# dalab/matrix-manifolds

Hardware: AMD Instinct MI355X
Metric: pairwise manifold-dist/sec (fwd+bwd), SPD(3) 5k-node (higher is better)
Workload: dtype f32; 1 GPU; grqc-class graph, n=5000 nodes -> SPD(3) affine-invariant, all 12497500 pairs, squared distance + backward, reference init (||log X||=0.1); parallelism=pair-rows sharded x1, 1 all-reduce, launch=hipGraph replay (kernels)

## Files before the change

matrix-manifolds_amd/csrc/spd_pair.hpp:

```cpp
#pragma once
#include <hip/hip_runtime.h>

#include "../../include/mm_manifolds.h"
#include "prof.hpp"
#include <algorithm>
#include <climits>
#include <cstdint>
#include <cstdlib>
#include <type_traits>

#include "smallmat.hpp"
#include "loss.hpp"
#include "adam.hpp"
#include "spd_rules.hpp"

#include "spd_ws.hpp"
#include "spd_step.hpp"
#include "stamp.hpp"

namespace mm {

template <typename T, int D>
__device__ __forceinline__ void node_tables(const T (&xs)[Packed<D>::NP], int i, T* __restrict__ nodeL, T* __restrict__ nodeX,
                                            T* __restrict__ nodeC, int* __restrict__ bad, T* __restrict__ nodeLd,
// ... 125 lines not shown
  }
  T s = T(0);
#pragma unroll
  for (int k = 0; k < D; ++k) {
    w[k] = Num<T>::min(Num<T>::max(ev[k], wmin), wmax);
    lw[k] = Num<T>::log(w[k]);
    s = Num<T>::fma(lw[k], lw[k], s);
    if (rho) rho[k] = w[k] == ev[k] ? T(1) : ev[k] * Num<T>::rcp(w[k]);
  }
  return s;
}

template <typename T, int D> __device__ __forceinline__ T frob2(const T (&m)[Packed<D>::NP]) {
  T s = T(0);
#pragma unroll
  for (int r = 0; r < D; ++r) {
    s = Num<T>::fma(m[pidx(r, r)], m[pidx(r, r)], s);
#pragma unroll
    for (int c = 0; c < r; ++c) s = Num<T>::fma(T(2) * m[pidx(r, c)], m[pidx(r, c)], s);
  }
  return s;
}
template <typename T, int D> __device__ __forceinline__ T close_gate(const T (&a)[Packed<D>::NP]) {
  using N = Num<T>;
  T e[Packed<D>::NP];
#pragma unroll
  for (int k = 0; k < Packed<D>::NP; ++k) e[k] = a[k];
#pragma unroll
  for (int r = 0; r < D; ++r) e[pidx(r, r)] -= T(1);
  if constexpr (D == 3) {
    return N::fma(e[0], e[0], N::fma(e[1], e[1], e[3] * e[3])) + N::fma(e[1], e[1], N::fma(e[2], e[2], e[4] * e[4])) +
           N::fma(e[3], e[3], N::fma(e[4], e[4], e[5] * e[5]));
  } else {
    T p2 = T(0);
#pragma unroll
    for (int r = 0; r < D; ++r) {
      T acc = e[pidx(r, 0)] * e[pidx(0, r)];
#pragma unroll
      for (int k = 1; k < D; ++k) acc = N::fma(e[pidx(r, k)], e[pidx(k, r)], acc);
      p2 += acc;
    }
    return p2;
  }
}
constexpr double kCloseGate = 0.09;
template <typename T, int D> __device__ __forceinline__ void log_close(const T (&a)[Packed<D>::NP], T (&m0)[Packed<D>::NP],
                                                                     T pre = T(1)) {
  if constexpr (D == 3) log_series3<T>(a, m0, pre); else log_series4<T>(a, m0, pre);
}
template <typename T, int D> __device__ __forceinline__ T log_cayley(const T (&a)[Packed<D>::NP], T (&m0)[Packed<D>::NP], T pre = T(1)) {
  if constexpr (D == 3) {
    return log_cayley3<T>(a, m0, pre);
  } else {
    const T gate = log_cayley4<T>(a, m0);
#pragma unroll
    for (int k = 0; k < Packed<D>::NP; ++k) m0[k] *= pre;
    return gate;
  }
}
template <typename T, int D> constexpr bool fwd_uses_logdet() {
  return D == 3 && std::is_same<T, double>::value;
}

__host__ __device__ inline bool spd_clamps_wide(double wmin, double wmax) { return wmin <= 1e-6 && wmax >= 1e6; }
template <int D, int LOSS> inline bool spd_clamps_supported(double wmin, double wmax) {
  return (D <= 2 && LOSS == MM_LOSS_NONE) || spd_clamps_wide(wmin, wmax);
}
template <typename T, int D, bool CHOL = false, bool HAS_LD = false, typename TL>
__device__ __forceinline__ T pair_value(const TL (&li)[Packed<D>::NP], const T (&xj)[Packed<D>::NP], T wmin, T wmax,
                                        T logdet_a = T(0)) {
  if constexpr (D == 3 && std::is_same<T, float>::value) {
    float a[6], w[3], v[3][3];
    pair_a<float, 3, CHOL>(li, xj, a);
    if (__builtin_expect(!__any(!(close_dev3<float>(a) <= float(kCloseGate))), 1)) {
      float e2;
      return logsq_series3<float>(a, &e2);
    }
    if (!__any(centred_far3<float>(a))) return logsq_series3_centred<float>(a);
    eig3_trig(a, w);
    const bool wide = !(w[0] * 32.f > w[2]);
    if (__any(wide)) {
      if constexpr (CHOL) {
        float lw[3];
        return pair_core<float, 3, false, true>(li, xj, wmin, wmax, w, lw, v);
      } else {
        jacobi_eig<float, 3, false, true>(a, v, Num<float>::eps());
        w[0] = a[pidx(0, 0)]; w[1] = a[pidx(1, 1)]; w[2] = a[pidx(2, 2)];
      }
    }
    float s = 0.f;
#pragma unroll
    for (int k = 0; k < 3; ++k) {
      const float l = Num<float>::log(fminf(fmaxf(w[k], wmin), wmax));
      s = fmaf(l, l, s);
    }
    return s;
  } else if constexpr (D == 3 || D == 4) {
    constexpr int NP = Packed<D>::NP;
    T a[NP], m0[NP];
    pair_a<T, D, CHOL>(li, xj, a);
    if constexpr (D == 3) {
      if (__builtin_expect(!__any(!(close_dev3<T>(a) <= T(kCloseGate))), 1)) {
        T e2;
        return logsq_series3<T>(a, &e2);
      }
      if constexpr (HAS_LD && fwd_uses_logdet<T, D>()) {
        T gate;
        const T sc = logsq_cayley3<T>(a, logdet_a, &gate);
        if (__builtin_expect(!__any(!(gate <= T(kCayleyGate))), 1)) return sc;
        T w[D], lw[D], v[D][D];
        return pair_core<T, D, false, CHOL>(li, xj, wmin, wmax, w, lw, v);
      }
    } else {
      if (__builtin_expect(!__any(!(close_gate<T, D>(a) <= T(kCloseGate))), 1)) return logsq_series4<T>(a);
      if constexpr (std::is_same<T, float>::value) {
        if (!__any(centred_far4<T>(a))) return logsq_series4_centred<T>(a);
      }
    }
    const T gate = log_cayley<T, D>(a, m0);
    if (__builtin_expect(!__any(!(gate <= T(kCayleyGate))), 1)) return frob2<T, D>(m0);
    T w[D], lw[D], v[D][D];
    return pair_core<T, D, false, CHOL>(li, xj, wmin, wmax, w, lw, v);
  } else if constexpr (D == 2 && CHOL) {
    T mlog[3];
    return log_pair2_chol<T>(li, xj, wmin, wmax, mlog);
  } else if constexpr (D >= 5) {
    constexpr int NP = Packed<D>::NP;
    T a[NP], m0[NP];
    pair_a<T, D, CHOL>(li, xj, a);
    if (__builtin_expect(!__any(!(close_gate<T, D>(a) <= T(kCloseGate))), 1)) {
      log_close_mat<T, D>(a, m0);
      return frob2<T, D>(m0);
    }
    if (!__any(centred_far_mat<T, D>(a))) {
      log_centred_mat<T, D>(a, m0);
      return frob2<T, D>(m0);
    }
    T w[D], lw[D], v[D][D];
    return pair_core<T, D, false, CHOL>(li, xj, wmin, wmax, w, lw, v);
  } else {
    T w[D], lw[D], v[D][D];
    return pair_core<T, D, false, CHOL>(li, xj, wmin, wmax, w, lw, v);
  }
}

constexpr int kSpd2FwdNC = 2, kSpd2BwdNC = 2;
template <typename T, int D> constexpr int pair_cols() { return (sizeof(T) == 4 && D == 2) ? kSpd2FwdNC : (sizeof(T) == 4 && D <= 3) ? 2 : ((sizeof(T) == 4 && D == 4) ? MM_SPD4_FWD_NC : 1); }
template <typename T, int D> constexpr int pair_cols_bwd() { return (sizeof(T) == 4 && D == 3) ? MM_SPD3_BWD_NC : (sizeof(T) == 4 && D == 2) ? kSpd2BwdNC : ((sizeof(T) == 4 && D == 4) ? MM_SPD4_BWD_NC : 1); }

template <typename T, int D, int TI, bool SQ>
__global__ __launch_bounds__(kBlock) void spd_pdist_fwd_kernel(const T* __restrict__ nodeL,
                                                               const T* __restrict__ nodeY ,
                                                               const T* __restrict__ nodeLd , int n, int row_begin,
                                                               int row_end, T wmin, T wmax, T* __restrict__ out) {
  constexpr int NP = Packed<D>::NP;
  constexpr int NC = pair_cols<T, D>();
  constexpr bool kLd = fwd_uses_logdet<T, D>();
  static_assert(TI % 2 == 0, "the row loop is unrolled twice");
  const TileId tile = fold_tile<TI, kBlock * NC>(n, row_begin, row_end);
  if (!tile.ok) return;
  const int i0 = tile.i0, i1 = min(i0 + TI, row_end);
  const int lane = threadIdx.x & 63;
  const int wave = __builtin_amdgcn_readfirstlane(threadIdx.x >> 6);
  const int wave_j0 = tile.jbase + wave * (64 * NC);
  if (wave_j0 + 64 * NC - 1 <= i0) return;
  int jv[NC];
  unsigned joff[NC];
  T xj[NC][NP], ldj[NC];
  static_for<NC>([&](auto qc) {
    constexpr int q = decltype(qc)::value;
    const int j = wave_j0 + 64 * q + lane;
    const bool jin = j < n;
    jv[q] = jin ? j : INT32_MIN;
    asm volatile("" : "+v"(jv[q]));
    joff[q] = unsigned(j) * unsigned(sizeof(T));
#pragma unroll
    for (int k = 0; k < NP; ++k) xj[q][k] = T(0);
#pragma unroll
    for (int k = 0; k < D; ++k) xj[q][pidx(k, k)] = T(1);
    ldj[q] = T(0);
    if (jin) {
#pragma unroll
      for (int k = 0; k < NP; ++k) xj[q][k] = nodeY[size_t(j) * NP + k];
      if constexpr (kLd) ldj[q] = nodeLd[j];
    }
  });
  const int64_t base = pair_off(n, row_begin);
  char* op = reinterpret_cast<char*>(out + (pair_off(n, i0) - base - i0 - 1));
  unsigned ostep = unsigned(n - i0 - 2) * unsigned(sizeof(T));
  unsigned roff = unsigned(i0) * unsigned(NP * sizeof(T));
  T lrow[2][NP], ldrow[2] = {T(0), T(0)};
#pragma unroll
  for (int k = 0; k < NP; ++k) lrow[0][k] = nodeL[size_t(i0) * NP + k];
  if constexpr (kLd) ldrow[0] = nodeLd[i0];
  const bool interior = wave_j0 >= i1 && wave_j0 + 64 * NC <= n && ((i1 - i0) & 1) == 0;
  auto row_loop = [&](auto masked_c) __attribute__((always_inline)) {
  constexpr bool kMasked = decltype(masked_c)::value;
  for (int ib = i0; ib < i1; ib += 2) {
#pragma unroll
    for (int u = 0; u < 2; ++u) {
      const int irow = ib + u;
      const int ieff = (u == 0 || irow < i1) ? irow : INT32_MAX;
      roff += unsigned(NP * sizeof(T));
      asm volatile("" : "+s"(roff));
      const T* rowp = reinterpret_cast<const T*>(reinterpret_cast<const char*>(nodeL) + roff);
#pragma unroll
      for (int k = 0; k < NP; ++k) lrow[u ^ 1][k] = rowp[k];
      if constexpr (kLd) ldrow[u ^ 1] = nodeLd[irow + 1];
      const T (&li)[NP] = lrow[u];
      static_for<NC>([&](auto qc) {
        constexpr int q = decltype(qc)::value;
        T s = Num<T>::max_raw_s(pair_value<T, D, true, kLd>(li, xj[q], wmin, wmax, ldj[q] - ldrow[u]), wmin);
        if constexpr (!SQ) s = Num<T>::sqrt(s);
        asm volatile("" : "+v"(joff[q]));
        if (!kMasked || jv[q] > ieff) *reinterpret_cast<T*>(op + joff[q]) = s;
      });
      op += ostep;
      ostep -= unsigned(sizeof(T));
    }
  }
  };
  if (interior) row_loop(std::false_type{}); else row_loop(std::true_type{});
}

template <typename T, int LOSS>
__device__ __forceinline__ T upstream_of(T loaded, T dsq, bool valid, int squared, T wmin, T sp, const LossArgs<T>& la,
                                         T& loss_acc, T& ds_acc) {
  if constexpr (LOSS == MM_LOSS_NONE) {
    if (__builtin_expect(!squared, 0)) loaded *= T(0.5) * Num<T>::rsqrt(Num<T>::max(dsq, wmin));
    return loaded;
  } else {
    T dldm;
    const T l = loss_term<T, LOSS>(sp * dsq, loaded, la, dldm);
    loss_acc += valid ? l : T(0);
    ds_acc += valid ? dldm * dsq : T(0);
    return valid ? dldm * sp : T(0);
  }
}

__device__ __forceinline__ int batch_node(const int* __restrict__ idx32, size_t k, int n_total) {
  return int(min(unsigned(idx32[2 * k]), unsigned(n_total - 1)));
}

template <typename T>
__device__ __forceinline__ T pair_row_load(const T* __restrict__ g, int n, int64_t base, int row, int j) {
  const char* grow = reinterpret_cast<const char*>(g + (pair_off(n, row) - base - row - 1));
  const unsigned off = unsigned(min(max(j, row + 1), n - 1)) * unsigned(sizeof(T));
  return *reinterpret_cast<const T*>(grow + off);
}

template <typename T, int D, int TI, int LOSS, bool SQ, int NCX = 0, bool SUB = false>
__global__ __launch_bounds__((64 * bwd_waves<T, D>()), (bwd_min_waves_nc<T, D, NCX>())) void spd_pdist_bwd_kernel(const T* __restrict__ nodeLC ,
                                                               const T* __restrict__ nodeY ,
                                                               const T* __restrict__ g, int n, int row_begin,
                                                               int row_end, T wmin, T wmax,
                                                               T* __restrict__ accM, T* __restrict__ accS,
                                                               LossArgs<T> la,
                                                               const int64_t* __restrict__ idx, int n_total,
                                                               WalkShares shares, int* __restrict__ share_tab) {
  static_assert(!SUB || LOSS != MM_LOSS_NONE, "node minibatches exist for the fused objective only");
  const int ns = SUB ? n_total : n;
  const int* idx32 = reinterpret_cast<const int*>(idx);
  constexpr int NP = Packed<D>::NP;
  constexpr int NW = bwd_waves<T, D>();
  constexpr int NC = NCX ? NCX : pair_cols_bwd<T, D>();
  constexpr int squared = SQ ? 1 : 0;
  T sp = T(1), loss_acc = T(0), ds_acc = T(0);
  loss_resolve<T, LOSS>(la);
  if constexpr (LOSS != MM_LOSS_NONE) sp = softplus_of(la.scale_raw);
  static_assert(TI % 2 == 0, "the row loop is unrolled twice");
  __shared__ T redM[NW][TI][NP];
  __shared__ T colS[NW][NC][D * D][64];
  MM_SPD_STAMP_BEGIN();
  __builtin_amdgcn_s_setprio(3);
  const ColWalk walk(n, row_begin, row_end, 64 * NC);
  int cb, r, rem;
  shares.of_cached(walk, int(blockIdx.x), share_tab, cb, r, rem);
  const int lane = threadIdx.x & 63;
  const int wave = __builtin_amdgcn_readfirstlane(threadIdx.x >> 6);
  bool red_writer;
  const int red_slot = reduce_slot<NP>(lane, red_writer);
  const int64_t base = pair_off(n, row_begin);
  MM_SPD_STAMP_MARK(0);
  const int wave_rows = (rem + NW - 1) / NW;
  constexpr int kPrioLast = 4;
  const int prio_last = max(kPrioLast, wave_rows / 10);
  const int prio_stretch = max(wave_rows - prio_last, 3) / 3;
  int rows_left = prio_stretch;
  int phase = 0;
  __shared__ T redJunk[NW][64];
  T* red_ptr = red_writer ? &redM[wave][0][red_slot] : &redJunk[wave][lane];
  const int red_step = red_writer ? NP : 0;

  while (rem > 0) {
    const int jbase = cb * (64 * NC);
    int jv[NC];
    unsigned joff[NC];
    T xj[NC][NP], accJ[NC][D][D];
    static_for<NC>([&](auto qc) {
      constexpr int q = decltype(qc)::value;
      const int j = jbase + 64 * q + lane;
      const bool jin = j < n;
      jv[q] = jin ? j : INT32_MIN;
      asm volatile("" : "+v"(jv[q]));
      joff[q] = unsigned(min(j, n - 1)) * unsigned(sizeof(T));
      int jn = j;
      if constexpr (SUB) {
        jn = batch_node(idx32, size_t(min(j, n - 1)), n_total);
        joff[q] = unsigned(jn) * unsigned(sizeof(T));
      }
#pragma unroll
      for (int k = 0; k < NP; ++k) xj[q][k] = T(0);
#pragma unroll
      for (int k = 0; k < D; ++k) xj[q][pidx(k, k)] = T(1);
      if (jin) {
#pragma unroll
        for (int k = 0; k < NP; ++k) xj[q][k] = nodeY[size_t(jn) * NP + k];
      }
#pragma unroll
      for (int rr = 0; rr < D; ++rr)
#pragma unroll
        for (int c = 0; c < D; ++c) accJ[q][rr][c] = T(0);
    });
    const int hi = walk.hi(cb);
    const int slice_cap = max(TI, int(min(int64_t(1) << 20, (int64_t(1) << 31) / (int64_t(n) * int64_t(sizeof(T))))));
    while (rem > 0 && r < hi) {
      const int chunk = int(min(int64_t(min(hi - r, rem)), int64_t(NW) * slice_cap));
      const int tw = (chunk + NW - 1) / NW;
      const int i0 = min(r + wave * tw, r + chunk), i1 = min(i0 + tw, r + chunk);
      if (i0 < i1) {
        constexpr int kAhead = 2;
        static_assert(kAhead == 2, "the one padding row of the operand table covers one masked slot: further ahead, clamp roff");
        const int first_node = SUB ? __builtin_amdgcn_readfirstlane(batch_node(idx32, size_t(i0), n_total)) : i0;
        int next_node = SUB ? __builtin_amdgcn_readfirstlane(batch_node(idx32, size_t(min(i0 + 1, n - 1)), n_total)) : 0;
        unsigned roff = unsigned(first_node) * unsigned(2 * NP * sizeof(T));
        T lrow[kAhead][2 * NP];
#pragma unroll
        for (int k = 0; k < 2 * NP; ++k) lrow[0][k] = nodeLC[size_t(first_node) * (2 * NP) + k];
        const int glast = min(i1, walk.re) - 1;
        const int64_t gk = glast - i0;
        const unsigned gmax = unsigned((gk * (n - 2) - (int64_t(i0) * gk + gk * (gk - 1) / 2)) * int64_t(sizeof(T)));
// ... 454 lines not shown
      const T lo = Num<T>::min(e[j], e[j + 1]), hi = Num<T>::max(e[j], e[j + 1]);
      e[j] = lo; e[j + 1] = hi;
    }
  if (in) {
#pragma unroll
    for (int r = 0; r < D; ++r) w[k * D + r] = e[r];
  }
}

template <typename T, int D>
__global__ void spd_rsgd_step_kernel(const T* x, const T* __restrict__ eg, int64_t m, T lr,
                                     T max_grad_norm, int exact, T* xnew) {
  constexpr int NP = Packed<D>::NP;
  const int64_t k0 = int64_t(blockIdx.x) * blockDim.x + threadIdx.x;
  const bool in = k0 < m;
  const int64_t k = in ? k0 : 0;
  T xs[NP], gs[NP], o[NP];
  load_sym_packed<T, D>(x + k * D * D, xs);
  load_sym_packed<T, D>(eg + k * D * D, gs);
  spd_rsgd_update<T, D>(xs, gs, lr, max_grad_norm, exact, o);
  if (in) store_sym_full<T, D>(xnew + k * D * D, o);
}

template <typename T, int D>
__global__ void spd_rsgd_momentum_kernel(const T* x, const T* __restrict__ eg, T* buf, int64_t m, T lr, T momentum,
                                         T dampening, T max_grad_norm, int exact, T* xnew) {
  constexpr int NP = Packed<D>::NP;
  const int64_t k0 = int64_t(blockIdx.x) * blockDim.x + threadIdx.x;
  const bool in = k0 < m;
  const int64_t k = in ? k0 : 0;
  T xs[NP], gs[NP], o[NP], b[NP];
  load_sym_packed<T, D>(x + k * D * D, xs);
  load_sym_packed<T, D>(eg + k * D * D, gs);
  load_sym_packed<T, D>(buf + k * D * D, b);
  spd_momentum_update<T, D>(xs, gs, b, lr, momentum, dampening, max_grad_norm, exact, o);
  if (in) {
    store_sym_full<T, D>(xnew + k * D * D, o);
    store_sym_full<T, D>(buf + k * D * D, b);
  }
}

template <typename T, int D>
__global__ void spd_radam_step_kernel(const T* x, const T* __restrict__ eg, T* exp_avg, T* exp_avg_sq, int64_t m,
                                      AdamArgs<T> a, T* xnew) {
  constexpr int NP = Packed<D>::NP;
  const int64_t k0 = int64_t(blockIdx.x) * blockDim.x + threadIdx.x;
  const bool in = k0 < m;
  const int64_t k = in ? k0 : 0;
  T beta2, alpha;
  adam_coeffs(a, beta2, alpha);
  T xs[NP], gs[NP], o[NP], mo[NP];
  load_sym_packed<T, D>(x + k * D * D, xs);
  load_sym_packed<T, D>(eg + k * D * D, gs);
  load_sym_packed<T, D>(exp_avg + k * D * D, mo);
  const T v = spd_adam_update<T, D>(xs, gs, mo, exp_avg_sq[k * D * D], a, beta2, alpha, o);
  if (in) {
    store_sym_full<T, D>(xnew + k * D * D, o);
    store_sym_full<T, D>(exp_avg + k * D * D, mo);
#pragma unroll
    for (int q = 0; q < D * D; ++q) exp_avg_sq[k * D * D + q] = v;
  }
  adam_tick(a.step, a.ticket, gridDim.x);
}

enum { RULE_RSGD = 0, RULE_MOMENTUM = 1, RULE_ADAM = 2 };
template <typename T> struct StepRule {
  T lr, momentum, dampening, max_grad_norm;
  int exact;
  T* state0;
  T* state1;
  AdamArgs<T> adam;
};
template <typename T> struct StepFuse {
  const T* nodeL; T* accM; T* accS;
  T* grad;
  T* slots; const T* scale_raw; T* loss_out;
  T* scale_x; T scale_lr, scale_clip;
  T* tabL; T* tabX; T* tabC; int* bad; T* tabLd; T* tabLC;
};
template <typename T, int D, int RULE, bool FIN, bool PREP>
__global__ void spd_fused_step_kernel(T* x, int n, StepRule<T> rule, StepFuse<T> f) {
  constexpr int NP = Packed<D>::NP;
  if constexpr (FIN) {
    if (f.slots && blockIdx.x == 0 && threadIdx.x < 64) {
      loss_finalize<T>(f.slots, f.scale_raw, f.loss_out);
      if (f.scale_x && threadIdx.x == 0) {
        const T g = f.loss_out[1];
        T scale = -f.scale_lr;
        if (f.scale_clip > T(0)) scale *= Num<T>::min(f.scale_clip / Num<T>::sqrt(Num<T>::max(g * g, T(1e-8))), T(1));
        *f.scale_x = *f.scale_x + g * scale;
      }
    }
  }
  const int i0 = blockIdx.x * blockDim.x + threadIdx.x;
  const bool in = i0 < n;
  const int i = in ? i0 : 0;
  T beta2 = T(0), alpha = T(0);
  if constexpr (RULE == RULE_ADAM) adam_coeffs(rule.adam, beta2, alpha);
  T xs[NP], gs[NP], o[NP];
  load_sym_packed<T, D>(x + size_t(i) * D * D, xs);
  if constexpr (FIN) {
    if (in) {
      node_gradient<T, D>(f.nodeL, f.accM, f.accS, n, i, gs);
      store_sym_full<T, D>(f.grad + size_t(i) * D * D, gs);
    } else {
#pragma unroll
      for (int k = 0; k < NP; ++k) gs[k] = T(0);
    }
  } else {
    load_sym_packed<T, D>(f.grad + size_t(i) * D * D, gs);
  }
  if constexpr (RULE == RULE_RSGD) {
    spd_rsgd_update<T, D>(xs, gs, rule.lr, rule.max_grad_norm, rule.exact, o);
  } else if constexpr (RULE == RULE_MOMENTUM) {
    T b[NP];
    load_sym_packed<T, D>(rule.state0 + size_t(i) * D * D, b);
    spd_momentum_update<T, D>(xs, gs, b, rule.lr, rule.momentum, rule.dampening, rule.max_grad_norm, rule.exact, o);
    if (in) store_sym_full<T, D>(rule.state0 + size_t(i) * D * D, b);
  } else {
    T mo[NP];
    load_sym_packed<T, D>(rule.state0 + size_t(i) * D * D, mo);
    const T v = spd_adam_update<T, D>(xs, gs, mo, rule.state1[size_t(i) * D * D], rule.adam, beta2, alpha, o);
    if (in) {
      store_sym_full<T, D>(rule.state0 + size_t(i) * D * D, mo);
#pragma unroll
      for (int q = 0; q < D * D; ++q) rule.state1[size_t(i) * D * D + q] = v;
    }
  }
  if (in) {
    store_sym_full<T, D>(x + size_t(i) * D * D, o);
    if constexpr (PREP) node_tables<T, D>(o, i, f.tabL, f.tabX, f.tabC, f.bad, f.tabLd, f.tabLC);
  }
  if constexpr (RULE == RULE_ADAM) adam_tick(rule.adam.step, rule.adam.ticket, gridDim.x);
}

#define MM_CHECK_LAUNCH()                         \
  do {                                            \
    hipError_t e_ = hipGetLastError();            \
    if (e_ != hipSuccess) return static_cast<int>(e_); \
  } while (0)

constexpr int kNodeBlock = 128;
template <typename T, int D>
int spd_pdist_prepare(const T* x, int64_t n, Ws<T>& ws, int flags, hipStream_t st) {
  if (!(flags & MM_WS_PREPARED)) {
    spd_prep_kernel<T, D><<<dim3((n + kNodeBlock - 1) / kNodeBlock), dim3(kNodeBlock), 0, st>>>(x, int(n), ws.nodeL, ws.nodeX, ws.nodeC,
                                                                       ws.accM, ws.accS, ws.loss, ws.bad, ws.nodeLd, ws.nodeLC);
    MM_CHECK_LAUNCH();
  }
  return MM_OK;
}

constexpr int kFwdTI = 8;
template <typename T, int D, int TI>
int spd_pdist_fwd_launch(const T* nl, const T* nc, const T* nld, int64_t n, int64_t rb, int64_t re, int squared, double wmin, double wmax,
                         T* out, hipStream_t st) {
  if (!spd_clamps_supported<D, MM_LOSS_NONE>(wmin, wmax)) return MM_ERR_UNSUPPORTED;
  const dim3 grid = fold_grid<TI, kBlock * pair_cols<T, D>()>(n, rb, re);
  if (squared)
    launch_timed(PROF_SPD_FWD, spd_pdist_fwd_kernel<T, D, TI, true>, grid, dim3(kBlock), st, nl, nc, nld, int(n), int(rb), int(re),
                 T(wmin), T(wmax), out);
  else
    launch_timed(PROF_SPD_FWD, spd_pdist_fwd_kernel<T, D, TI, false>, grid, dim3(kBlock), st, nl, nc, nld, int(n), int(rb), int(re),
                 T(wmin), T(wmax), out);
  MM_CHECK_LAUNCH();
  return MM_OK;
}
template <typename T, int D>
int spd_pdist_fwd_t(const T* x, int64_t n, int64_t rb, int64_t re, int squared, double wmin, double wmax, T* out,
                    void* wsp, int flags, hipStream_t st) {
  Ws<T> ws(wsp, n, D);
  int rc = spd_pdist_prepare<T, D>(x, n, ws, flags, st);
  if (rc) return rc;
  if (re <= rb || pair_off(n, re) == pair_off(n, rb)) return MM_OK;
  const T* nl = ws.nodeL;
  const T* nc = ws.nodeC;
  if constexpr (D <= 4) {
    const dim3 g8 = fold_grid<kFwdTI, kBlock * pair_cols<T, D>()>(n, rb, re);
    if (int64_t(g8.x) * g8.y < 4 * int64_t(device_cus()))
      return spd_pdist_fwd_launch<T, D, 2>(nl, nc, ws.nodeLd, n, rb, re, squared, wmin, wmax, out, st);
  }
  return spd_pdist_fwd_launch<T, D, kFwdTI>(nl, nc, ws.nodeLd, n, rb, re, squared, wmin, wmax, out, st);
}

constexpr int kBwdTI = 16;
template <typename T> constexpr int bwd_cross_units() { return sizeof(T) == 4 ? 16 : 8; }
constexpr int64_t kSpd4TwoColPairs = 30000000;
constexpr int64_t kSpd4TwoColBandPairs = 12000000;
template <typename T, int D, int LOSS, bool SQ, int NCX = 0, bool SUB = false>
int spd_pdist_bwd_launch_sq(Ws<T>& ws, const T* g, int64_t n, int64_t rb, int64_t re, double wmin, double wmax,
                            hipStream_t st, LossArgs<T> la, const int64_t* idx = nullptr, int64_t n_total = 0) {
  if (!spd_clamps_supported<D, LOSS>(wmin, wmax)) return MM_ERR_UNSUPPORTED;
  constexpr int kThreads = 64 * bwd_waves<T, D>();
  constexpr int kCols = NCX ? NCX : pair_cols_bwd<T, D>();
  if constexpr (!SUB && NCX == 0 && sizeof(T) == 4 && D == 4 && pair_cols_bwd<T, D>() == 1) {
    static const int two = [] { const char* e = std::getenv("MM_SPD4_BWD_TWO_COLS"); return e ? (e[0] == '1' ? 1 : 0) : -1; }();
    const int64_t pairs = pair_off(n, re) - pair_off(n, rb);
    if (two == 1 || (two < 0 && (pairs >= kSpd4TwoColPairs || (pairs >= kSpd4TwoColBandPairs && re + 2048 <= n))))
      return spd_pdist_bwd_launch_sq<T, D, LOSS, SQ, 2>(ws, g, n, rb, re, wmin, wmax, st, la);
  }
  auto kernel = spd_pdist_bwd_kernel<T, D, kBwdTI, LOSS, SQ, NCX, SUB>;
  const int64_t units = ColWalk(int(n), int(rb), int(re), 64 * kCols).total();
  if (units <= 0) return MM_OK;
  int64_t grid = resident_workgroups<spd_pdist_bwd_kernel<T, D, kBwdTI, LOSS, SQ, NCX, SUB>>(kThreads);
  {
    const int64_t cus = device_cus();
    grid = std::min<int64_t>(grid, 4 * cus);
    const int64_t half = std::max<int64_t>(1, cus / 2);
    const int64_t by_rows = kCols >= 2 ? (units / 32 + half / 2) / half * half : units / 48 / cus * cus;
    if (by_rows < grid) grid = std::max<int64_t>(cus, by_rows);
  }
  static const int64_t env_grid = std::getenv("MM_SPD_BWD_GRID") ? std::atoll(std::getenv("MM_SPD_BWD_GRID")) : 0;
  if (env_grid > 0) grid = env_grid;
  grid = std::max<int64_t>(1, std::min<int64_t>(grid, (units + 7) / 8));
  dim3 g3{unsigned(grid), 1, 1};
  const T* nlc = ws.nodeLC;
  const T* nc = ws.nodeC;
  static const int env_cross = std::getenv("MM_SPD_BWD_CROSS") ? std::atoi(std::getenv("MM_SPD_BWD_CROSS")) : bwd_cross_units<T>();
  const ColWalk hw(int(n), int(rb), int(re), 64 * kCols);
  const int cross = std::min(std::max(env_cross, 0), 1024);
  const WalkShares shares(hw.total_aug(cross), grid, cross);
  launch_timed(PROF_SPD_BWD, kernel, g3, dim3(kThreads), st, nlc, nc, g, int(n), int(rb), int(re), T(wmin), T(wmax), ws.accM, ws.accS, la,
               idx, int(n_total), shares, ws.shareTab);
  MM_CHECK_LAUNCH();
  return MM_OK;
}
template <typename T, int D, int LOSS = MM_LOSS_NONE>
int spd_pdist_bwd_launch(Ws<T>& ws, const T* g, int64_t n, int64_t rb, int64_t re, int squared, double wmin, double wmax,
                         hipStream_t st, LossArgs<T> la = LossArgs<T>{nullptr, T(1), T(0), 0, nullptr}) {
  if constexpr (LOSS != MM_LOSS_NONE) return spd_pdist_bwd_launch_sq<T, D, LOSS, true>(ws, g, n, rb, re, wmin, wmax, st, la);
  else return squared ? spd_pdist_bwd_launch_sq<T, D, LOSS, true>(ws, g, n, rb, re, wmin, wmax, st, la)
                      : spd_pdist_bwd_launch_sq<T, D, LOSS, false>(ws, g, n, rb, re, wmin, wmax, st, la);
}

template <typename T, int D>
int spd_pdist_loss_t(int kind, const T* x, const T* target, const T* scale_raw, int64_t n, int64_t rb, int64_t re,
                     double alpha, double eps, int terms, const double* loss_params, double wmin, double wmax, T* loss_out, T* grad, void* wsp,
                     int flags, hipStream_t st) {
  Ws<T> ws(wsp, n, D);
  int rc = spd_pdist_prepare<T, D>(x, n, ws, flags, st);
  if (rc) return rc;
  if (re > rb && pair_off(n, re) > pair_off(n, rb)) {
    LossArgs<T> la{scale_raw, T(alpha), T(eps), terms, ws.loss, loss_params};
    if (kind == MM_LOSS_STRESS) rc = spd_pdist_bwd_launch<T, D, MM_LOSS_STRESS>(ws, target, n, rb, re, 1, wmin, wmax, st, la);
    else rc = spd_pdist_bwd_launch<T, D, MM_LOSS_QUOTIENT>(ws, target, n, rb, re, 1, wmin, wmax, st, la);
    if (rc) return rc;
  }
  spd_pdist_finalize_kernel<T, D><<<dim3((n + kNodeBlock - 1) / kNodeBlock), dim3(kNodeBlock), 0, st>>>(ws.nodeL, ws.accM, ws.accS, int(n),
                                                                               grad, ws.loss, scale_raw, loss_out);
  MM_CHECK_LAUNCH();
  return MM_OK;
}

template <typename T, int D>
int spd_pdist_loss_subset_t(int kind, const T* x, const T* dense, const T* scale_raw, int64_t n_total, const int64_t* idx, int64_t bs,
                            int64_t rb, int64_t re, double alpha, double eps, int terms, const double* loss_params, double wmin,
                            double wmax, T* loss_out, T* grad, void* wsp, int flags, hipStream_t st) {
  Ws<T> ws(wsp, n_total, D);
  int rc = spd_pdist_prepare<T, D>(x, n_total, ws, flags, st);
  if (rc) return rc;
  if (re > rb && pair_off(bs, re) > pair_off(bs, rb)) {
    LossArgs<T> la{scale_raw, T(alpha), T(eps), terms, ws.loss, loss_params};
    if (kind == MM_LOSS_STRESS)
      rc = spd_pdist_bwd_launch_sq<T, D, MM_LOSS_STRESS, true, 0, true>(ws, dense, bs, rb, re, wmin, wmax, st, la, idx, n_total);
    else
      rc = spd_pdist_bwd_launch_sq<T, D, MM_LOSS_QUOTIENT, true, 0, true>(ws, dense, bs, rb, re, wmin, wmax, st, la, idx, n_total);
    if (rc) return rc;
  }
  spd_pdist_finalize_kernel<T, D><<<dim3((n_total + kNodeBlock - 1) / kNodeBlock), dim3(kNodeBlock), 0, st>>>(ws.nodeL, ws.accM, ws.accS, int(n_total),
                                                                                     grad, ws.loss, scale_raw, loss_out);
  MM_CHECK_LAUNCH();
  return MM_OK;
}

template <typename T, int D>
int spd_pdist_bwd_t(const T* x, const T* g, int64_t n, int64_t rb, int64_t re, int squared, double wmin, double wmax,
                    T* grad, void* wsp, int flags, hipStream_t st) {
  constexpr int NP = Packed<D>::NP;
  Ws<T> ws(wsp, n, D);
  int rc = spd_pdist_prepare<T, D>(x, n, ws, flags, st);
  if (rc) return rc;
  if (re > rb && pair_off(n, re) > pair_off(n, rb)) {
    rc = spd_pdist_bwd_launch<T, D>(ws, g, n, rb, re, squared, wmin, wmax, st);
    if (rc) return rc;
  }
  spd_pdist_finalize_kernel<T, D><<<dim3((n + kNodeBlock - 1) / kNodeBlock), dim3(kNodeBlock), 0, st>>>(
      ws.nodeL, ws.accM, ws.accS, int(n), grad, static_cast<T*>(nullptr), static_cast<const T*>(nullptr),
      static_cast<T*>(nullptr));
  MM_CHECK_LAUNCH();
  return MM_OK;
}

template <typename T, int D, bool FIN>
int spd_fused_step_launch(const mm_train_step* s, Ws<T>& ws, hipStream_t st, bool fuse_scale) {
  const mm_step_param& p = s->points[0];
  const mm_step_param& q = s->scales[0];
  const int n = int(s->n);
  StepRule<T> rule{T(p.lr), T(p.momentum), T(p.dampening), T(p.max_grad_norm), p.exact, static_cast<T*>(p.state0),
                   static_cast<T*>(p.state1),
                   AdamArgs<T>{T(p.lr), T(p.beta1), T(p.beta2), T(p.adam_eps), T(p.max_grad_norm), p.nc, p.exact, p.step, p.ticket}};
  StepFuse<T> f{ws.nodeL, ws.accM, ws.accS, static_cast<T*>(p.grad),
                ws.loss, static_cast<const T*>(q.x), static_cast<T*>(s->loss_out),
                fuse_scale ? static_cast<T*>(q.x) : nullptr, T(q.lr), T(q.max_grad_norm),
                ws.nodeL, ws.nodeX, ws.nodeC, ws.bad, ws.nodeLd, ws.nodeLC};
  const dim3 grid((n + 127) / 128), block(128);
  T* x = static_cast<T*>(p.x);
  if (p.optimizer == MM_OPT_RADAM) spd_fused_step_kernel<T, D, RULE_ADAM, FIN, true><<<grid, block, 0, st>>>(x, n, rule, f);
  else if (p.momentum != 0.0) spd_fused_step_kernel<T, D, RULE_MOMENTUM, FIN, true><<<grid, block, 0, st>>>(x, n, rule, f);
  else spd_fused_step_kernel<T, D, RULE_RSGD, FIN, true><<<grid, block, 0, st>>>(x, n, rule, f);
  MM_CHECK_LAUNCH();
  return MM_OK;
}

template <typename T, int D, bool SUB = false>
int spd_fused_train_step_t(const mm_train_step* s, int64_t rb, int64_t re, bool with_objective, hipStream_t st,
                           bool* scale_stepped) {
  const int64_t n = s->n;
  Ws<T> ws(s->ws, n, D);
  *scale_stepped = false;
  if (!with_objective) return spd_fused_step_launch<T, D, false>(s, ws, st, false);
  int rc = spd_pdist_prepare<T, D>(static_cast<const T*>(s->points[0].x), n, ws, s->ws_flags, st);
  if (rc) return rc;
  const int64_t np = SUB ? s->batch : n;
  if (re > rb && pair_off(np, re) > pair_off(np, rb)) {
    LossArgs<T> la{static_cast<const T*>(s->scales[0].x), T(s->alpha), T(s->eps), s->terms, ws.loss, s->loss_params};
    const T* target = static_cast<const T*>(s->target);
    if constexpr (SUB) {
      if (s->loss_kind == MM_LOSS_STRESS)
        rc = spd_pdist_bwd_launch_sq<T, D, MM_LOSS_STRESS, true, 0, true>(ws, target, np, rb, re, s->wmin, s->wmax, st, la, s->batch_idx, n);
      else
        rc = spd_pdist_bwd_launch_sq<T, D, MM_LOSS_QUOTIENT, true, 0, true>(ws, target, np, rb, re, s->wmin, s->wmax, st, la, s->batch_idx, n);
    } else {
      if (s->loss_kind == MM_LOSS_STRESS)
        rc = spd_pdist_bwd_launch<T, D, MM_LOSS_STRESS>(ws, target, n, rb, re, 1, s->wmin, s->wmax, st, la);
      else
// ... 39 lines not shown
```

matrix-manifolds_amd/csrc/spd_ws.hpp:

```cpp
#pragma once
#include <hip/hip_runtime.h>

#include <atomic>
#include <cstdint>

#include "../../include/mm_manifolds.h"
#include "loss.hpp"
#include "smallmat.hpp"

namespace mm {

constexpr int kBlock = 256;
constexpr int64_t kSpdMaxNodes = int64_t(1) << 22;
#ifndef MM_SPD4_BWD_WAVES
#define MM_SPD4_BWD_WAVES 4
#endif
#ifndef MM_SPD4_BWD_NC
#define MM_SPD4_BWD_NC 1
#endif
#ifndef MM_SPD4_FWD_NC
#define MM_SPD4_FWD_NC 1
#endif
#ifndef MM_SPD3_BWD_NC
#define MM_SPD3_BWD_NC 2
#endif
#ifndef MM_SPD3_BWD_WAVES
#define MM_SPD3_BWD_WAVES 4
#endif
#ifndef MM_SPD3_F64_BWD_WAVES
#define MM_SPD3_F64_BWD_WAVES 3
#endif
template <typename T, int D> constexpr int bwd_min_waves() {
  return (sizeof(T) == 4 && D == 3) ? MM_SPD3_BWD_WAVES : ((sizeof(T) == 4 && D == 4) ? MM_SPD4_BWD_WAVES : ((sizeof(T) == 8 && D == 3) ? MM_SPD3_F64_BWD_WAVES : 1));
}
#ifndef MM_SPD4_BWD2_WAVES
#define MM_SPD4_BWD2_WAVES 3
#endif
template <typename T, int D, int NCX> constexpr int bwd_min_waves_nc() {
  return (NCX == 2 && sizeof(T) == 4 && D == 4) ? MM_SPD4_BWD2_WAVES : bwd_min_waves<T, D>();
}
template <typename T, int D> constexpr int bwd_waves() {
  return int(sizeof(T)) * D * D * 64 * 4 <= 65536 ? 4 : (int(sizeof(T)) * D * D * 64 * 2 <= 65536 ? 2 : 1);
}
#ifndef MM_SPD_MAX_D
#define MM_SPD_MAX_D 9
#endif
constexpr int kSpdMaxD = MM_SPD_MAX_D;

__host__ __device__ inline int64_t pair_off(int64_t n, int64_t row) { return row * (2 * n - row - 1) / 2; }

constexpr int kShareTabEntries = 2048;
inline size_t vec_ws_tables_end(size_t esz, int64_t n, int mp) {
  return (esz * (size_t(n) * (mp + 1) + 2 * kLossSlots + size_t(n + 1) * mp) + 31) / 32 * 32;
}
template <typename T> struct Ws {
  int* status;
  int* bad;
  T* nodeL;
  T* nodeX;
  T* nodeC;
  T* accM;
  T* accS;
  T* loss;
  T* nodeLd;
  T* nodeLC;
  int* shareTab;
  static size_t bad_bytes(int64_t n) { return (size_t(n) * sizeof(int) + 63) / 64 * 64; }
  static size_t tables_end(int64_t n, int d) {
    const int np = d * (d + 1) / 2;
    return 64 + bad_bytes(n) + sizeof(T) * (size_t(n) * (6 * np + d * d + 1) + 2 * kLossSlots + 2 * np);
  }
  static size_t bytes(int64_t n, int d) { return (tables_end(n, d) + 31) / 32 * 32 + size_t(kShareTabEntries) * 32; }
  Ws(void* base, int64_t n, int d) {
    const int np = d * (d + 1) / 2;
    char* p = static_cast<char*>(base);
    status = reinterpret_cast<int*>(p);
    bad = reinterpret_cast<int*>(p + 64);
    nodeL = reinterpret_cast<T*>(p + 64 + bad_bytes(n));
    nodeX = nodeL + n * np;
    nodeC = nodeX + n * np;
    accM = nodeC + n * np;
    accS = accM + n * np;
    loss = accS + n * d * d;
    nodeLd = loss + 2 * kLossSlots;
    nodeLC = nodeLd + n;
    shareTab = reinterpret_cast<int*>(p + (tables_end(n, d) + 31) / 32 * 32);
  }
};

struct TileId { int i0, jbase; bool ok; };
template <int TI, int BW = kBlock> __device__ __forceinline__ TileId fold_tile(int n, int row_begin, int row_end) {
  const int gy = (row_end - row_begin + TI - 1) / TI;
  const int nJB = (n + BW - 1) / BW;
  int y = blockIdx.y, x = blockIdx.x;
  int cb0 = (row_begin + y * TI + 1) / BW;
  int cnt = nJB - cb0;
  if (x >= cnt) {
    x -= cnt;
    const int y2 = gy - 1 - y;
    if (y2 <= y) return {0, 0, false};
    y = y2;
    cb0 = (row_begin + y * TI + 1) / BW;
    cnt = nJB - cb0;
    if (x >= cnt) return {0, 0, false};
  }
  return {row_begin + y * TI, (cb0 + x) * BW, true};
}
template <int TI, int BW = kBlock> inline dim3 fold_grid(int64_t n, int64_t rb, int64_t re) {
  const int gy = int((re - rb + TI - 1) / TI);
  const int nJB = int((n + BW - 1) / BW);
  int gx = 0;
  for (int y = 0; y < (gy + 1) / 2; ++y) {
    const int y2 = gy - 1 - y;
    int c = nJB - int((rb + int64_t(y) * TI + 1) / BW);
    if (y2 > y) c += nJB - int((rb + int64_t(y2) * TI + 1) / BW);
    gx = c > gx ? c : gx;
  }
  return dim3(gx > 0 ? gx : 1, (gy + 1) / 2 > 0 ? (gy + 1) / 2 : 1);
}


struct ColWalk {
  int rb, re, ncb, c0, c1, bw;
  __host__ __device__ ColWalk(int n, int row_begin, int row_end, int block_width = 64) {
    bw = block_width;
    rb = row_begin;
    re = row_end < n - 1 ? row_end : n - 1;
    if (re < rb) re = rb;
    ncb = (n + bw - 1) / bw;
    c0 = (rb + 1) / bw;
    c1 = re / bw > c0 ? re / bw : c0;
    if (c1 > ncb) c1 = ncb;
    if (c0 > ncb) c0 = ncb;
  }
  __host__ __device__ int hi(int c) const { const int d = bw * c + bw - 1; return d < re ? d : re; }
  __host__ __device__ int64_t prefix(int c) const {
    if (c <= c0 || re == rb) return 0;
    const int64_t m = c < c1 ? c : c1;
    int64_t s = (bw / 2) * (m * (m - 1) - int64_t(c0) * (c0 - 1)) + (m - c0) * int64_t(bw - 1 - rb);
    if (c > c1) s += int64_t(c - c1) * (re - rb);
    return s;
  }
  __host__ __device__ int64_t total() const { return prefix(ncb); }
  __host__ __device__ int find(int64_t p) const {
    int lo = c0, hi_ = ncb - 1;
    while (lo < hi_) {
      const int mid = (lo + hi_ + 1) / 2;
      if (prefix(mid) <= p) lo = mid; else hi_ = mid - 1;
    }
    return lo;
  }
  static __host__ __device__ void divmod_small(int64_t total, int64_t g, int64_t& q, int64_t& r) {
    q = int64_t(double(total) / double(g));
    r = total - q * g;
    if (r < 0) { --q; r += g; } else if (r >= g) { ++q; r -= g; }
  }
  static __host__ __device__ int64_t share_begin(int64_t total, int64_t w, int64_t g) {
    int64_t q, r;
    divmod_small(total, g, q, r);
    return q * w + (w < r ? w : r);
  }
  __host__ __device__ int find_fast(int64_t p, int cross = 0) const {
    int64_t off;
    return find_fast_off(p, cross, &off);
  }
  __host__ __device__ int find_fast_off(int64_t p, int cross, int64_t* off, bool* capped = nullptr) const {
    const int last = ncb - 1;
    if (capped) *capped = false;
    if (last <= c0) { *off = p; return c0; }
    int c;
    const int64_t pc1 = aprefix(c1, cross);
    if (p >= pc1) {
      const float R = float(re - rb + cross);
      c = c1 + int(float(p - pc1) / (R > 0.f ? R : 1.f));
    } else {
      const float A = 0.5f * float(bw), Bs = A - 1.0f + float(bw * c0 - rb + cross);
      c = c0 + int((-Bs + sqrtf(Bs * Bs + 4.0f * A * float(p))) / (2.0f * A));
    }
    c = c < c0 ? c0 : (c > last ? last : c);
    int64_t P = aprefix(c, cross);
    int ku = 0, kd = 0;
    for (; ku < 4 && c < last; ++ku) {
      const int64_t L = int64_t(hi(c) - rb + cross);
      if (P + L > p) break;
      P += L;
      ++c;
    }
    for (; kd < 4 && c > c0 && P > p; ++kd) {
      --c;
      P -= int64_t(hi(c) - rb + cross);
    }
    if (__builtin_expect(ku == 4 || kd == 4, 0)) {
      if (capped) *capped = true;
      int lo = c0, hi_ = last;
#pragma nounroll
      while (lo < hi_) {
        const int mid = (lo + hi_ + 1) / 2;
        if (aprefix(mid, cross) <= p) lo = mid; else hi_ = mid - 1;
      }
      c = lo;
      P = aprefix(c, cross);
    }
    *off = p - P;
    return c;
  }
  __host__ __device__ bool find_fast_converges(int64_t p, int cross = 0) const {
    int64_t off;
    bool capped;
    find_fast_off(p, cross, &off, &capped);
    return !capped;
  }
  __host__ __device__ int64_t aprefix(int c, int cross) const { return prefix(c) + int64_t(cross) * (c > c0 ? c - c0 : 0); }
  __host__ __device__ int64_t total_aug(int cross) const { return total() + int64_t(cross) * (ncb > c0 ? ncb - c0 : 0); }
  __host__ __device__ void enter(int64_t a, int count, int cross, int* block, int* row, int* left) const {
    int64_t off;
    const int c = find_fast_off(a, cross, &off);
    *block = c;
    if (off < cross) { *row = rb; *left = count - int(cross - off); }
    else { *row = rb + int(off - cross); *left = count; }
  }
};

struct WalkShares {
  int64_t q;
  int r;
  int cross;
  WalkShares() = default;
  WalkShares(int64_t units, int64_t grid, int cross_ = 0) : q(units / grid), r(int(units % grid)), cross(cross_) {}
  __device__ __forceinline__ void of(int w, int64_t& begin, int& count) const {
    begin = q * int64_t(w) + (w < r ? w : r);
    count = int(q) + (w < r ? 1 : 0);
  }
  __device__ __forceinline__ void of(const ColWalk& walk, int w, int& block, int& row, int& left) const {
    int64_t a;
    int cnt;
    of(w, a, cnt);
    walk.enter(a, cnt, cross, &block, &row, &left);
  }
  __device__ __forceinline__ void of_cached(const ColWalk& walk, int w, int* __restrict__ tab, int& block, int& row, int& left) const {
    const bool usable = tab != nullptr && w < kShareTabEntries && r < (1 << 18) && q < (int64_t(1) << 31) && walk.ncb < (1 << 16);
    const int k4 = (r << 13) | (cross << 2) | ((walk.bw >> 6) - 1);
    const int k2 = walk.ncb | (w << 16);
    if (usable) {
      const int* e = tab + 8 * w;
      const int e0 = e[0], e1 = e[1], e2 = e[2], e3 = e[3], e4 = e[4], e5 = e[5], e6 = e[6], e7 = e[7];
      if (e0 == walk.rb && e1 == walk.re && e2 == k2 && e3 == int(q) && e4 == k4) {
        block = e5;
        row = e6;
        left = e7;
        return;
      }
    }
    of(walk, w, block, row, left);
    if (usable && threadIdx.x == 0) {
      int* e = tab + 8 * w;
      e[5] = block; e[6] = row; e[7] = left;
      e[0] = walk.rb; e[1] = walk.re; e[2] = k2; e[3] = int(q); e[4] = k4;
    }
  }
};

inline int device_cus() {
  static int cache[64] = {0};
  int dev = 0;
  if (hipGetDevice(&dev) != hipSuccess || dev < 0 || dev >= 64) dev = 0;
  if (cache[dev] == 0) {
    int cus = 0;
    if (hipDeviceGetAttribute(&cus, hipDeviceAttributeMultiprocessorCount, dev) != hipSuccess || cus < 1) cus = 256;
    cache[dev] = cus;
  }
  return cache[dev];
}

// ... 17 lines not shown
```

Before: 169.7 billion pairs/s.

## Use variable-height row tiles in SPD forward pairwise-distance kernel

Replaces the fixed TI-row folded tiling of the forward pairwise kernel with a host-built schedule of up to four runs of tile heights (16/8/4/2). Heights are chosen from the remaining work per resident workgroup, or from an environment rule. The goal is tall tiles for row reuse early and short tiles at the tail, so the last wave of blocks stays balanced, replacing the old TI=2 fallback. It adds per-block tile decoding arithmetic and a host-side cache of the schedule keyed on (n, rb, re, resident).

```diff
diff --git a/matrix-manifolds_amd/csrc/spd_pair.hpp b/matrix-manifolds_amd/csrc/spd_pair.hpp
--- a/matrix-manifolds_amd/csrc/spd_pair.hpp
+++ b/matrix-manifolds_amd/csrc/spd_pair.hpp
@@ -301,14 +301,14 @@
 __global__ __launch_bounds__(kBlock) void spd_pdist_fwd_kernel(const T* __restrict__ nodeL,
                                                                const T* __restrict__ nodeY ,
                                                                const T* __restrict__ nodeLd , int n, int row_begin,
-                                                               int row_end, T wmin, T wmax, T* __restrict__ out) {
+                                                               int row_end, T wmin, T wmax, T* __restrict__ out, FwdTiles tiles) {
   constexpr int NP = Packed<D>::NP;
   constexpr int NC = pair_cols<T, D>();
   constexpr bool kLd = fwd_uses_logdet<T, D>();
   static_assert(TI % 2 == 0, "the row loop is unrolled twice");
-  const TileId tile = fold_tile<TI, kBlock * NC>(n, row_begin, row_end);
+  const FwdTile tile = fwd_tile<kBlock * NC>(tiles, n, row_begin, row_end, int(blockIdx.x), int(blockIdx.y));
   if (!tile.ok) return;
-  const int i0 = tile.i0, i1 = min(i0 + TI, row_end);
+  const int i0 = tile.i0, i1 = min(i0 + tile.rows, row_end);
   const int lane = threadIdx.x & 63;
   const int wave = __builtin_amdgcn_readfirstlane(threadIdx.x >> 6);
   const int wave_j0 = tile.jbase + wave * (64 * NC);
@@ -334,8 +334,8 @@
       if constexpr (kLd) ldj[q] = nodeLd[j];
     }
   });
-  const int64_t base = pair_off(n, row_begin);
-  char* op = reinterpret_cast<char*>(out + (pair_off(n, i0) - base - i0 - 1));
+  const int64_t row_off = int64_t((uint64_t(unsigned(i0)) * uint64_t(unsigned(2 * n - i0 - 1))) >> 1);
+  char* op = reinterpret_cast<char*>(out + (row_off - tiles.base - i0 - 1));
   unsigned ostep = unsigned(n - i0 - 2) * unsigned(sizeof(T));
   unsigned roff = unsigned(i0) * unsigned(NP * sizeof(T));
   T lrow[2][NP], ldrow[2] = {T(0), T(0)};
@@ -1096,17 +1096,32 @@
 }
 
 constexpr int kFwdTI = 8;
-template <typename T, int D, int TI>
+inline const FwdTileRule& fwd_tile_rule() {
+  static const FwdTileRule rule = FwdTileRule::parse(std::getenv("MM_SPD_FWD_TILES"));
+  return rule;
+}
+template <typename T, int D>
 int spd_pdist_fwd_launch(const T* nl, const T* nc, const T* nld, int64_t n, int64_t rb, int64_t re, int squared, double wmin, double wmax,
                          T* out, hipStream_t st) {
   if (!spd_clamps_supported<D, MM_LOSS_NONE>(wmin, wmax)) return MM_ERR_UNSUPPORTED;
-  const dim3 grid = fold_grid<TI, kBlock * pair_cols<T, D>()>(n, rb, re);
+  if (re > n - 1) re = n - 1;
+  const int resident = squared ? resident_workgroups<spd_pdist_fwd_kernel<T, D, kFwdTI, true>>(kBlock)
+                               : resident_workgroups<spd_pdist_fwd_kernel<T, D, kFwdTI, false>>(kBlock);
+  struct Key { int64_t n, rb, re; int resident; };
+  thread_local Key last_key = {-1, -1, -1, -1};
+  thread_local FwdTiles last_tiles;
+  thread_local dim3 last_grid;
+  if (last_key.n != n || last_key.rb != rb || last_key.re != re || last_key.resident != resident) {
+    last_tiles = fwd_tiles_build<kBlock * pair_cols<T, D>()>(n, rb, re, resident, fwd_tile_rule(), &last_grid);
+    last_key = {n, rb, re, resident};
+  }
+  const dim3 grid = last_grid;
   if (squared)
-    launch_timed(PROF_SPD_FWD, spd_pdist_fwd_kernel<T, D, TI, true>, grid, dim3(kBlock), st, nl, nc, nld, int(n), int(rb), int(re),
-                 T(wmin), T(wmax), out);
+    launch_timed(PROF_SPD_FWD, spd_pdist_fwd_kernel<T, D, kFwdTI, true>, grid, dim3(kBlock), st, nl, nc, nld, int(n), int(rb), int(re),
+                 T(wmin), T(wmax), out, last_tiles);
   else
-    launch_timed(PROF_SPD_FWD, spd_pdist_fwd_kernel<T, D, TI, false>, grid, dim3(kBlock), st, nl, nc, nld, int(n), int(rb), int(re),
-                 T(wmin), T(wmax), out);
+    launch_timed(PROF_SPD_FWD, spd_pdist_fwd_kernel<T, D, kFwdTI, false>, grid, dim3(kBlock), st, nl, nc, nld, int(n), int(rb), int(re),
+                 T(wmin), T(wmax), out, last_tiles);
   MM_CHECK_LAUNCH();
   return MM_OK;
 }
@@ -1117,14 +1132,7 @@
   int rc = spd_pdist_prepare<T, D>(x, n, ws, flags, st);
   if (rc) return rc;
   if (re <= rb || pair_off(n, re) == pair_off(n, rb)) return MM_OK;
-  const T* nl = ws.nodeL;
-  const T* nc = ws.nodeC;
-  if constexpr (D <= 4) {
-    const dim3 g8 = fold_grid<kFwdTI, kBlock * pair_cols<T, D>()>(n, rb, re);
-    if (int64_t(g8.x) * g8.y < 4 * int64_t(device_cus()))
-      return spd_pdist_fwd_launch<T, D, 2>(nl, nc, ws.nodeLd, n, rb, re, squared, wmin, wmax, out, st);
-  }
-  return spd_pdist_fwd_launch<T, D, kFwdTI>(nl, nc, ws.nodeLd, n, rb, re, squared, wmin, wmax, out, st);
+  return spd_pdist_fwd_launch<T, D>(ws.nodeL, ws.nodeC, ws.nodeLd, n, rb, re, squared, wmin, wmax, out, st);
 }
 
 constexpr int kBwdTI = 16;
diff --git a/matrix-manifolds_amd/csrc/spd_ws.hpp b/matrix-manifolds_amd/csrc/spd_ws.hpp
--- a/matrix-manifolds_amd/csrc/spd_ws.hpp
+++ b/matrix-manifolds_amd/csrc/spd_ws.hpp
@@ -3,6 +3,9 @@
 
 #include <atomic>
 #include <cstdint>
+#include <cstdio>
+#include <cstdlib>
+#include <cstring>
 
 #include "../../include/mm_manifolds.h"
 #include "loss.hpp"
@@ -119,6 +122,113 @@
   return dim3(gx > 0 ? gx : 1, (gy + 1) / 2 > 0 ? (gy + 1) / 2 : 1);
 }
 
+struct FwdTiles {
+  int y0[4];
+  int c[4];
+  int h[4];
+  int64_t base;
+};
+struct FwdTile { int i0, rows, jbase; bool ok; };
+template <int BW> __host__ __device__ __forceinline__ FwdTile fwd_tile(const FwdTiles& s, int n, int rb, int re, int bx, int by) {
+  const int R = re - rb, nJB = (n + BW - 1) / BW;
+  int Ha = s.c[0] + s.h[0] * by, Hb = s.c[0] + s.h[0] * (by + 1);
+#define MM_FWD_TILE_LINE(k) \
+  { const int la = s.c[k] + s.h[k] * by, lb = s.c[k] + s.h[k] * (by + 1); Ha = la < Ha ? la : Ha; Hb = lb < Hb ? lb : Hb; }
+  MM_FWD_TILE_LINE(1) MM_FWD_TILE_LINE(2) MM_FWD_TILE_LINE(3)
+#undef MM_FWD_TILE_LINE
+  const int h = Hb - Ha;
+  const int rem = R - 2 * Ha;
+  int a = Ha, b = rem > h ? Hb : Ha + ((rem + 1) >> 1);
+  if (b <= a) return {0, 0, 0, false};
+  int cb0 = (rb + a + 1) / BW, cnt = nJB - cb0;
+  if (bx >= cnt) {
+    bx -= cnt;
+    a = R - Hb > b ? R - Hb : b;
+    b = R - Ha;
+    if (b <= a) return {0, 0, 0, false};
+    cb0 = (rb + a + 1) / BW;
+    cnt = nJB - cb0;
+    if (bx >= cnt) return {0, 0, 0, false};
+  }
+  return {rb + a, b - a, (cb0 + bx) * BW, true};
+}
+struct FwdTileRule {
+  int runs = 0;
+  int h[4] = {0, 0, 0, 0};
+  double frac[4] = {0, 0, 0, 0};
+  double t16 = 8.0, t8 = 4.0, t4 = 2.0;
+  static FwdTileRule parse(const char* e) {
+    FwdTileRule r, dflt;
+    if (e == nullptr || *e == 0) return dflt;
+    if (std::strncmp(e, "rule:", 5) == 0) {
+      if (std::sscanf(e + 5, "%lf,%lf,%lf", &r.t16, &r.t8, &r.t4) != 3 || !(r.t16 >= r.t8 && r.t8 >= r.t4 && r.t4 >= 0)) return dflt;
+      return r;
+    }
+    const char* p = e;
+    while (*p && r.runs < 4) {
+      char* q = nullptr;
+      const long hh = std::strtol(p, &q, 10);
+      if (q == p || (hh != 16 && hh != 8 && hh != 4 && hh != 2) || (r.runs > 0 && hh > r.h[r.runs - 1])) return dflt;
+      double f = 1.0;
+      p = q;
+      if (*p == ':') {
+        f = std::strtod(p + 1, &q);
+        if (q == p + 1 || !(f >= 0.0 && f <= 1.0)) return dflt;
+        p = q;
+      }
+      r.h[r.runs] = int(hh);
+      r.frac[r.runs] = f;
+      ++r.runs;
+      if (*p == ',') ++p; else if (*p) return dflt;
+    }
+    return (*p == 0 && r.runs > 0) ? r : dflt;
+  }
+};
+template <int BW> inline FwdTiles fwd_tiles_build(int64_t n, int64_t rb, int64_t re, int64_t resident, const FwdTileRule& rule, dim3* grid) {
+  FwdTiles s;
+  for (int k = 0; k < 4; ++k) { s.y0[k] = INT32_MAX; s.c[k] = 1 << 29; s.h[k] = 0; }
+  s.y0[0] = 0; s.c[0] = 0; s.h[0] = 2;
+  s.base = pair_off(n, rb);
+  if (re > n - 1) re = n - 1;
+  const int64_t R = re - rb, nJB = (n + BW - 1) / BW;
+  auto F = [](int64_t m) { const int64_t q = m / BW, r = m % BW; return int64_t(BW) * (q * (q - 1) / 2) + q * r; };
+  double left = R > 0 ? double(R * nJB - (F(re + 1) - F(rb + 1))) : 0.0;
+  const double slots = double(resident > 0 ? resident : 1);
+  int64_t quota = rule.runs > 0 ? int64_t(rule.frac[0] * double(R) / double(2 * rule.h[0]) + 0.5) : 0;
+  int run = -1, fk = 0, y = 0;
+  int64_t H = 0, gx = 1;
+  while (2 * H < R) {
+    int h;
+    if (rule.runs > 0) {
+      while (quota <= 0 && fk + 1 < rule.runs) { ++fk; quota = int64_t(rule.frac[fk] * double(R) / double(2 * rule.h[fk]) + 0.5); }
+      h = rule.h[fk];
+      --quota;
+    } else {
+      const double t = left / slots;
+      h = t > rule.t16 ? 16 : (t > rule.t8 ? 8 : (t > rule.t4 ? 4 : 2));
+    }
+    if (run < 0 || h != s.h[run]) {
+      ++run;
+      s.y0[run] = y; s.c[run] = int(H) - h * y; s.h[run] = h;
+    }
+    const int64_t rem = R - 2 * H, t1 = rem > h ? H + h : H + (rem + 1) / 2;
+    int64_t c = nJB - (rb + H + 1) / BW;
+    double cells = double((t1 - H) * c);
+    const int64_t b0 = R - H - h > t1 ? R - H - h : t1, b1 = R - H;
+    if (b1 > b0) {
+      const int64_t cb = nJB - (rb + b0 + 1) / BW;
+      c += cb;
+      cells += double((b1 - b0) * cb);
+    }
+    gx = c > gx ? c : gx;
+    left -= cells;
+    H += h;
+    ++y;
+  }
+  *grid = dim3(unsigned(gx), unsigned(y > 0 ? y : 1));
+  return s;
+}
+
 
 struct ColWalk {
   int rb, re, ncb, c0, c1, bw;
```

Result: no change. 169.9 billion pairs/s, median of 3 (+0.1%).
